# KatherLab/STAMP

Measured on AMD Instinct MI355X. Metric: tiles/sec encoded (224x224, ViT-L/14), higher is better.
Workload: dtype f16

## Files before the change

stamp_amd/csrc/attention_vit257.hip:

```cpp
#include "common.h"
#include <type_traits>

namespace amds {

constexpr int A7_KP = 256, A7_VS = 576;
constexpr int A7_K_BYTES = A7_KP * 128, A7_V_BYTES = 64 * A7_VS + 8 * 16, A7_T_BYTES = 3 * 64 * 4 + 128;
constexpr int A7_BUF = A7_K_BYTES + A7_V_BYTES + A7_T_BYTES;
constexpr int A7_PART = 68;
constexpr int A7_SCRATCH = 16 + 8 * 64 + 2 * 9 * A7_PART * 4;
constexpr int A7_OUT = 8 * 2048;
constexpr int A7_LDS = 2 * A7_BUF + A7_SCRATCH + A7_OUT;

#ifdef A7_TRACE
__device__ unsigned long long a7_trace[32 * 8 * 8];
#define A7_MARK(k)                                                                                            \
    do {                                                                                                      \
        if (blockIdx.x == 0 && lane == 0 && trace_it < 32) a7_trace[(trace_it * 8 + (k)) * 8 + wave] = __builtin_amdgcn_s_memtime(); \
    } while (0)
#else
#define A7_MARK(k) do { } while (0)
#endif

template <typename T>
__global__ void __launch_bounds__(512) attn_vit257_kernel(const T* __restrict__ qkv, T* __restrict__ out, int H, int n_items) {
    typedef typename Act<T>::vec8 vec8;
    typedef typename Act<T>::vec4 vec4;
    constexpr int Tn = 257, KP = A7_KP, VS = A7_VS;
    extern __shared__ __attribute__((aligned(16))) char smem[];
    char* sZero = smem + 2 * A7_BUF;
    char* sPw = sZero + 16;
    float* sPart = reinterpret_cast<float*>(sPw + 8 * 64);

    const int tid = threadIdx.x, lane = tid & 63;
    const int wave = __builtin_amdgcn_readfirstlane(tid >> 6);
    const int l31 = lane & 31, hi = lane >> 5;
    const int Dm = H * 64;
    const long ld = 3L * Dm;
    const float sc = 0.125f * 1.44269504088896340736f;
    const int swz = (l31 >> 1) & 7;

    struct Part { u32x4 k; u32x2 v0, v1; };
    Part pa, pb;
    T tq = (T)0.f, tk = (T)0.f, tv = (T)0.f;
    vec8 qn[4];
    const int ldb = (int)ld * 2;
    const int vu = tid >> 1, vhalf = tid & 1;
    const int voff_k = (tid >> 3) * ldb + Dm * 2 + (tid & 7) * 16;
    const int voff_v = (vu >> 3) * 2 * ldb + Dm * 4 + (vu & 7) * 16 + vhalf * 8;
    const int voff_q = (wave * 32 + l31) * ldb + hi * 16;
    const int lk_off = (tid >> 3) * 128 + (((tid & 7) ^ ((tid >> 4) & 7)) << 4);
    const int vk0 = (vu >> 3) * 2;
    const int lv_off = A7_K_BYTES + ((vu & 7) * 8 + vhalf * 4) * VS + (vu & 7) * 16 + ((vk0 & ~12) | ((vk0 & 4) << 1) | ((vk0 & 8) >> 1)) * 2;
    auto part_load = [&](Part& pt, __amdgpu_buffer_rsrc_t rs, int c) {
#if defined(A7_ABL) && (A7_ABL & 2)
        if (c >= 0) return;
#endif
        pt.k = __builtin_amdgcn_raw_buffer_load_b128(rs, voff_k, c * 64 * ldb, 0);
        pt.v0 = __builtin_amdgcn_raw_buffer_load_b64(rs, voff_v, c * 64 * ldb, 0);
        pt.v1 = __builtin_amdgcn_raw_buffer_load_b64(rs, voff_v, c * 64 * ldb + ldb, 0);
    };
    auto part_store = [&](const Part& pt, char* buf, int c) {
        *reinterpret_cast<u32x4*>(buf + lk_off + c * 64 * 128) = pt.k;
        typedef T vec4t __attribute__((ext_vector_type(4)));
        typedef T vec2 __attribute__((ext_vector_type(2)));
        const vec4t a = __builtin_bit_cast(vec4t, pt.v0), b2 = __builtin_bit_cast(vec4t, pt.v1);
#pragma unroll
        for (int e = 0; e < 4; ++e) {
            vec2 w;
            w[0] = a[e]; w[1] = b2[e];
            *reinterpret_cast<vec2*>(buf + lv_off + e * VS + c * 128) = w;
        }
    };
    auto rest_load = [&](__amdgpu_buffer_rsrc_t rs) {
#pragma unroll
        for (int ks = 0; ks < 4; ++ks) qn[ks] = __builtin_bit_cast(vec8, __builtin_amdgcn_raw_buffer_load_b128(rs, voff_q + ks * 32, 0, 0));
        tq = __builtin_bit_cast(T, __builtin_amdgcn_raw_buffer_load_b16(rs, lane * 2, KP * ldb, 0));
        tk = __builtin_bit_cast(T, __builtin_amdgcn_raw_buffer_load_b16(rs, lane * 2, KP * ldb + Dm * 2, 0));
        tv = __builtin_bit_cast(T, __builtin_amdgcn_raw_buffer_load_b16(rs, lane * 2, KP * ldb + Dm * 4, 0));
    };
    auto rest_store = [&](char* buf) {
        float* sT = reinterpret_cast<float*>(buf + A7_K_BYTES + A7_V_BYTES);
        if (tid < 64) {
            sT[tid] = Act<T>::to_f32(tk); sT[64 + tid] = Act<T>::to_f32(tv); sT[128 + tid] = Act<T>::to_f32(tq);
            reinterpret_cast<T*>(sT + 192)[tid] = tq;
        }
    };
    auto item_rsrc = [&](int item) {
        const int b = item / H, h = item - b * H;
        return __builtin_amdgcn_make_buffer_rsrc(const_cast<T*>(qkv + (long)b * Tn * ld + h * 64), 0, Tn * ldb, 0x00020000);
    };

    int item = blockIdx.x;
    if (item >= n_items) return;
    if (tid < 4) reinterpret_cast<float*>(sZero)[tid] = 0.f;
    auto merge_odd = [&](int pbuf, int it) {
        const float* pp = sPart + pbuf * 9 * A7_PART;
        float m = pp[64];
#pragma unroll
        for (int j = 1; j < 9; ++j) m = fmaxf(m, pp[j * A7_PART + 64]);
        float lsum = 0.f, ov = 0.f;
#pragma unroll
        for (int j = 0; j < 9; ++j) {
            const float w = __builtin_amdgcn_exp2f(pp[j * A7_PART + 64] - m);
            lsum = fmaf(w, pp[j * A7_PART + 65], lsum);
            ov = fmaf(w, pp[j * A7_PART + lane], ov);
        }
        const int b = it / H, h = it - b * H;
        out[((long)b * Tn + KP) * Dm + h * 64 + lane] = Act<T>::from_f32(ov / lsum);
    };
    {
        const __amdgpu_buffer_rsrc_t rs = item_rsrc(item);
        rest_load(rs);
#pragma unroll
        for (int c = 0; c < 4; c += 2) {
            part_load(pa, rs, c);
            part_load(pb, rs, c + 1);
            part_store(pa, smem, c);
            part_store(pb, smem, c + 1);
        }
        rest_store(smem);
    }
    vec8 qf[4];
#pragma unroll
    for (int ks = 0; ks < 4; ++ks) qf[ks] = qn[ks];
    __syncthreads();

    int cur = 0;
#ifdef A7_TRACE
    int trace_it = 0;
#endif
#pragma unroll 1
    for (; item < n_items; item += gridDim.x) {
        const int b = item / H, h = item - b * H;
        const char* sK = smem + cur * A7_BUF;
        const char* sVt = sK + A7_K_BYTES;
        const float* sKt = reinterpret_cast<const float*>(sK + A7_K_BYTES + A7_V_BYTES);
        const float* sVl = sKt + 64;
        const float* sQt = sKt + 128;
        const bool has_next = item + (int)gridDim.x < n_items;
        A7_MARK(0);
        if (wave == 0 && item != (int)blockIdx.x) merge_odd(cur ^ 1, item - (int)gridDim.x);
        const __amdgpu_buffer_rsrc_t nrs = item_rsrc(has_next ? item + (int)gridDim.x : item);
        A7_MARK(1);

        {
            f32x16 o[2];
#pragma unroll
            for (int dt = 0; dt < 2; ++dt)
#pragma unroll
                for (int r = 0; r < 16; ++r) o[dt][r] = 0.f;
            float mrun = -INFINITY, l = 0.f;
            const f32x16 zero16 = {0.f, 0.f, 0.f, 0.f, 0.f, 0.f, 0.f, 0.f, 0.f, 0.f, 0.f, 0.f, 0.f, 0.f, 0.f, 0.f};
            auto stage = [&](auto has_pv_c, auto has_qk_c, int c, float alpha_prev, f32x16 (&sc_)[2], vec8 (&pout)[2][2], const vec8 (&pprev)[2][2],
                             f32x16 (&sn)[2]) {
                constexpr bool HP = decltype(has_pv_c)::value, HQ = decltype(has_qk_c)::value;
                vec8 opnd[4];
                auto ld = [&](int i) {
                    if (i < 0 || i >= 16) return;
#if defined(A7_ABL) && (A7_ABL & 4)
                    if (i >= 0) { asm volatile("" : "+v"(opnd[i & 3])); return; }
#endif
                    if (i < 8) {
                        if (!HQ) return;
                        const int t = i & 1, ks = i >> 1;
                        opnd[i & 3] = *reinterpret_cast<const vec8*>(sK + (((c + 1) * 2 + t) * 32 + l31) * 128 + (((ks * 2 + hi) ^ swz) << 4));
                    } else {
                        if (!HP) return;
                        const int q = i - 8, t = q >> 2, ks = (q >> 1) & 1, dt = q & 1;
                        const int pos = ((c - 1) * 2 + t) * 32 + ks * 16 + hi * 8, d = dt * 32 + l31;
                        opnd[i & 3] = *reinterpret_cast<const vec8*>(sVt + d * VS + (d >> 3) * 16 + pos * 2);
                    }
                };
                auto mf = [&](int i) {
#if defined(A7_ABL) && (A7_ABL & 8)
                    if (i >= 0) { asm volatile("" : "+v"(sn[i & 1]), "+v"(o[i & 1]) : "v"(opnd[i & 3])); return; }
#endif
                    if (i < 8) {
                        if (!HQ) return;
                        const int t = i & 1, ks = i >> 1;
                        sn[t] = Act<T>::mfma32(opnd[i & 3], qf[ks], ks == 0 ? zero16 : sn[t]);
                    } else {
                        if (!HP) return;
                        const int q = i - 8, t = q >> 2, ks = (q >> 1) & 1, dt = q & 1;
                        o[dt] = Act<T>::mfma32(opnd[i & 3], pprev[t][ks], o[dt]);
                    }
                };
                float mx = -INFINITY, mnew = 0.f, alpha = 0.f, ls = 0.f;
#ifndef A7_LD_DIST
#define A7_LD_DIST 2
#endif
#pragma unroll
                for (int i = 0; i < A7_LD_DIST; ++i) ld(i);
#pragma unroll
                for (int sl = 0; sl < 16; ++sl) {
                    ld(sl + A7_LD_DIST);
                    mf(sl);
                    if (sl < 2) {
#pragma unroll
                        for (int f = 16 * sl; f < 16 * sl + 16; ++f) mx = fmaxf(mx, sc_[f >> 4][f & 15]);
                    }
                    if (sl == 2) {
                        mx = fmaxf(mx, __shfl_xor(mx, 32, 64));
                        mnew = fmaxf(mrun, mx * sc);
                        alpha = __builtin_amdgcn_exp2f(mrun - mnew);
                        mrun = mnew;
                    }
                    if ((sl == 2 || sl == 3) && HP) {
#pragma unroll
                        for (int r = 0; r < 16; ++r) o[sl - 2][r] *= alpha_prev;
                    }
                    if (sl >= 3 && sl < 14) {
#pragma unroll
                        for (int f = 3 * (sl - 3); f < 3 * (sl - 3) + 3 && f < 32; ++f) {
#if defined(A7_ABL) && (A7_ABL & 1)
                            const float pw = fmaf(sc_[f >> 4][f & 15], sc, -mnew);
#else
                            const float pw = __builtin_amdgcn_exp2f(fmaf(sc_[f >> 4][f & 15], sc, -mnew));
#endif
                            ls += pw;
                            pout[f >> 4][(f >> 3) & 1][f & 7] = Act<T>::from_f32(pw);
                        }
                    }
                    if (sl == 14) l = l * alpha + ls;
                    __builtin_amdgcn_sched_barrier(0);
                }
                return alpha;
            };
            typedef std::true_type Y;
            typedef std::false_type N_;
            char* nbuf = smem + (cur ^ 1) * A7_BUF;
            f32x16 sa[2], sb[2];
            vec8 p0[2][2], p1[2][2];
            part_load(pa, nrs, 0);
#pragma unroll
            for (int t = 0; t < 2; ++t) {
                sa[t] = zero16;
#pragma unroll
                for (int ks = 0; ks < 4; ++ks) {
                    const vec8 kf = *reinterpret_cast<const vec8*>(sK + (t * 32 + l31) * 128 + (((ks * 2 + hi) ^ swz) << 4));
                    sa[t] = Act<T>::mfma32(kf, qf[ks], sa[t]);
                }
            }
            __builtin_amdgcn_sched_barrier(0);
            part_load(pb, nrs, 1);
            __builtin_amdgcn_sched_barrier(0);
            const float al0 = stage(N_{}, Y{}, 0, 0.f, sa, p0, p1, sb);
            part_store(pa, nbuf, 0);
            part_load(pa, nrs, 2);
            __builtin_amdgcn_sched_barrier(0);
            const float al1 = stage(Y{}, Y{}, 1, al0, sb, p1, p0, sa);
            part_store(pb, nbuf, 1);
            part_load(pb, nrs, 3);
            __builtin_amdgcn_sched_barrier(0);
            const float al2 = stage(Y{}, Y{}, 2, al1, sa, p0, p1, sb);
            rest_load(nrs);
            __builtin_amdgcn_sched_barrier(0);
            const float al3 = stage(Y{}, N_{}, 3, al2, sb, p1, p0, sa);
#pragma unroll
            for (int dt = 0; dt < 2; ++dt)
#pragma unroll
                for (int r = 0; r < 16; ++r) o[dt][r] *= al3;
#pragma unroll
            for (int i = 0; i < 8; ++i) {
                const int t = i >> 2, ks = (i >> 1) & 1, dt = i & 1;
                const int pos = (6 + t) * 32 + ks * 16 + hi * 8, d = dt * 32 + l31;
                const vec8 vf = *reinterpret_cast<const vec8*>(sVt + d * VS + (d >> 3) * 16 + pos * 2);
                o[dt] = Act<T>::mfma32(vf, p1[t][ks], o[dt]);
            }
            A7_MARK(2);
            {
                float dot = 0.f;
#pragma unroll
                for (int ks = 0; ks < 4; ++ks) {
                    const f32x4 k0 = *reinterpret_cast<const f32x4*>(sKt + (ks * 2 + hi) * 8), k1 = *reinterpret_cast<const f32x4*>(sKt + (ks * 2 + hi) * 8 + 4);
#pragma unroll
                    for (int e = 0; e < 4; ++e) dot = fmaf(Act<T>::to_f32(qf[ks][e]), k0[e], fmaf(Act<T>::to_f32(qf[ks][4 + e]), k1[e], dot));
                }
                dot += __shfl_xor(dot, 32, 64);
                const float st = dot * sc, mnew = fmaxf(mrun, st);
                const float alpha = __builtin_amdgcn_exp2f(mrun - mnew), pt = __builtin_amdgcn_exp2f(st - mnew);
                mrun = mnew;
                l = l * alpha + (hi == 0 ? pt : 0.f);
#pragma unroll
                for (int dt = 0; dt < 2; ++dt)
#pragma unroll
                    for (int g = 0; g < 4; ++g) {
                        const f32x4 vv = *reinterpret_cast<const f32x4*>(sVl + dt * 32 + 8 * g + 4 * hi);
#pragma unroll
                        for (int e = 0; e < 4; ++e) o[dt][4 * g + e] = fmaf(o[dt][4 * g + e], alpha, pt * vv[e]);
                    }
            }
            l += __shfl_xor(l, 32, 64);
            const float inv = 1.0f / l;
            char* so = smem + 2 * A7_BUF + A7_SCRATCH + wave * 2048;
            T* obase = out + ((long)b * Tn + wave * 32) * Dm + h * 64;
#pragma unroll
            for (int r = 0; r < 2; ++r) {
                if ((l31 >> 4) == r) {
#pragma unroll
                    for (int dt = 0; dt < 2; ++dt)
#pragma unroll
                        for (int g = 0; g < 4; ++g) {
                            vec4 w;
#pragma unroll
                            for (int e = 0; e < 4; ++e) w[e] = Act<T>::from_f32(o[dt][4 * g + e] * inv);
                            *reinterpret_cast<vec4*>(so + (l31 & 15) * 128 + (((dt * 4 + g) ^ (l31 & 7)) << 4) + hi * 8) = w;
                        }
                }
                asm volatile("" ::: "memory");
#pragma unroll
                for (int k = 0; k < 2; ++k) {
                    const int row = k * 8 + (lane >> 3), c = lane & 7;
                    const u32x4 v = *reinterpret_cast<const u32x4*>(so + row * 128 + ((c ^ (row & 7)) << 4));
#if defined(A7_ABL) && (A7_ABL & 16)
                    if (n_items < 0)
#endif
                    *reinterpret_cast<u32x4*>(obase + (long)(r * 16 + row) * Dm + c * 8) = v;
                }
                asm volatile("" ::: "memory");
            }
        }

        A7_MARK(3);
        {
            const char* sQh = reinterpret_cast<const char*>(sKt + 192);
            const char* qsrc = l31 == 0 ? sQh + hi * 16 : sZero;
            const int qstep = l31 == 0 ? 32 : 0;
            f32x16 s1;
#pragma unroll
            for (int r = 0; r < 16; ++r) s1[r] = 0.f;
#pragma unroll
            for (int ks = 0; ks < 4; ++ks) {
                const vec8 qa = *reinterpret_cast<const vec8*>(qsrc + ks * qstep);
                const vec8 kf = *reinterpret_cast<const vec8*>(sK + (wave * 32 + l31) * 128 + (((ks * 2 + hi) ^ swz) << 4));
                s1 = Act<T>::mfma32(qa, kf, s1);
            }
            vec8 vfo[2][2];
#pragma unroll
            for (int ks = 0; ks < 2; ++ks)
#pragma unroll
                for (int dt = 0; dt < 2; ++dt) {
                    const int pos = wave * 32 + ks * 16 + hi * 8, d = dt * 32 + l31;
                    vfo[ks][dt] = *reinterpret_cast<const vec8*>(sVt + d * VS + (d >> 3) * 16 + pos * 2);
                }
            const float sv = hi == 0 ? s1[0] * sc : -INFINITY;
            const float mw = half_wave_max(sv);
            const float pk = hi == 0 ? __builtin_amdgcn_exp2f(sv - mw) : 0.f;
            const float lw = half_wave_sum(pk);
            char* pw = sPw + wave * 64;
            if (hi == 0) reinterpret_cast<T*>(pw)[(l31 & ~12) | ((l31 & 4) << 1) | ((l31 & 8) >> 1)] = Act<T>::from_f32(pk);
            asm volatile("" ::: "memory");
            const char* psrc = l31 == 0 ? pw + hi * 16 : sZero;
            f32x16 oq[2];
#pragma unroll
            for (int dt = 0; dt < 2; ++dt)
#pragma unroll
                for (int r = 0; r < 16; ++r) oq[dt][r] = 0.f;
#pragma unroll
            for (int ks = 0; ks < 2; ++ks) {
                const vec8 pf = *reinterpret_cast<const vec8*>(psrc + ks * qstep);
#pragma unroll
                for (int dt = 0; dt < 2; ++dt) oq[dt] = Act<T>::mfma32(vfo[ks][dt], pf, oq[dt]);
            }
            float* pp = sPart + (cur * 9 + wave) * A7_PART;
            if (l31 == 0) {
#pragma unroll
                for (int dt = 0; dt < 2; ++dt)
#pragma unroll
                    for (int g = 0; g < 4; ++g)
                        *reinterpret_cast<f32x4*>(pp + dt * 32 + 8 * g + 4 * hi) = f32x4{oq[dt][4 * g], oq[dt][4 * g + 1], oq[dt][4 * g + 2], oq[dt][4 * g + 3]};
                if (hi == 0) { pp[64] = mw; pp[65] = lw; }
            }
            if (wave == 1) {
                float* p8 = sPart + (cur * 9 + 8) * A7_PART;
                float st = half_wave_sum(sQt[lane] * sKt[lane]);
                st = (st + __shfl_xor(st, 32, 64)) * sc;
                p8[lane] = sVl[lane];
                if (lane == 0) { p8[64] = st; p8[65] = 1.0f; }
            }
        }

        A7_MARK(4);
        {
            char* nbuf = smem + (cur ^ 1) * A7_BUF;
            part_store(pa, nbuf, 2);
            part_store(pb, nbuf, 3);
            rest_store(nbuf);
#pragma unroll
            for (int ks = 0; ks < 4; ++ks) qf[ks] = qn[ks];
        }
        A7_MARK(5);
        __syncthreads();
        A7_MARK(6);
        cur ^= 1;
#ifdef A7_TRACE
        ++trace_it;
#endif
    }
    if (wave == 0) merge_odd(cur ^ 1, item - (int)gridDim.x);
}


template <typename T>
static int launch_attn257(const void* qkv, void* out, int B, int H, hipStream_t st) {
    auto kern = attn_vit257_kernel<T>;
    static bool attr_set = false;
    if (!attr_set) {
        AMDS_HIP(hipFuncSetAttribute(reinterpret_cast<const void*>(kern), hipFuncAttributeMaxDynamicSharedMemorySize, A7_LDS));
        attr_set = true;
    }
    const int n_cus = device_cu_count();
    AMDS_REQUIRE(n_cus > 0, "attention: cannot read the device's multiprocessor count");
    const int n_items = B * H;
    hipLaunchKernelGGL(kern, dim3(min(n_items, n_cus)), dim3(512), A7_LDS, st, (const T*)qkv, (T*)out, H, n_items);
    AMDS_LAUNCH_CHECK("attn_vit257_kernel");
    return AMDS_OK;
}

int attention_vit257(const void* qkv, void* out, int B, int H, int dtype, hipStream_t st) {
    return dtype == AMDS_F16 ? launch_attn257<f16>(qkv, out, B, H, st) : launch_attn257<bf16>(qkv, out, B, H, st);
}

}
```

Measured before the change: 6057.

## Load K/V straight to LDS and read V transposed with ds_read_b64_tr_b16

Replaces the register-staged K/V prefetch, which loaded into VGPRs and then wrote a manually transposed V layout to LDS, with direct buffer-to-LDS loads (bufl16) using an XOR-swizzled row layout for both K and V. The PV MFMA operands are then fetched with ds_read_b64_tr_b16 transpose reads, using per-lane addresses that flip between the double buffers each iteration. This removes the VGPR staging and the scalar-pair transpose stores, and with them some register pressure and LDS write traffic. In exchange it adds explicit vmcnt/lgkmcnt waits before each barrier and inline-asm reads that each wait on lgkmcnt(0), which may serialize LDS latency inside the pipelined stages.

```diff
diff --git a/stamp_amd/csrc/attention_vit257.hip b/stamp_amd/csrc/attention_vit257.hip
--- a/stamp_amd/csrc/attention_vit257.hip
+++ b/stamp_amd/csrc/attention_vit257.hip
@@ -3,8 +3,8 @@
 
 namespace amds {
 
-constexpr int A7_KP = 256, A7_VS = 576;
-constexpr int A7_K_BYTES = A7_KP * 128, A7_V_BYTES = 64 * A7_VS + 8 * 16, A7_T_BYTES = 3 * 64 * 4 + 128;
+constexpr int A7_KP = 256;
+constexpr int A7_K_BYTES = A7_KP * 128, A7_V_BYTES = A7_KP * 128, A7_T_BYTES = 3 * 64 * 4 + 128;
 constexpr int A7_BUF = A7_K_BYTES + A7_V_BYTES + A7_T_BYTES;
 constexpr int A7_PART = 68;
 constexpr int A7_SCRATCH = 16 + 8 * 64 + 2 * 9 * A7_PART * 4;
@@ -21,11 +21,22 @@
 #define A7_MARK(k) do { } while (0)
 #endif
 
+__device__ __forceinline__ int a7_swz(int row) { return (((row >> 1) & 1) << 2) | ((row >> 2) & 3); }
+
+#define A7_TR8(out, a00, a01, a10, a11, imm)                                                                                              \
+    asm volatile("ds_read_b64_tr_b16 %0, %8 offset:%12\n\tds_read_b64_tr_b16 %1, %10 offset:%12\n\t"                                  \
+                 "ds_read_b64_tr_b16 %2, %9 offset:%12\n\tds_read_b64_tr_b16 %3, %11 offset:%12\n\t"                                   \
+                 "ds_read_b64_tr_b16 %4, %8 offset:%13\n\tds_read_b64_tr_b16 %5, %10 offset:%13\n\t"                                   \
+                 "ds_read_b64_tr_b16 %6, %9 offset:%13\n\tds_read_b64_tr_b16 %7, %11 offset:%13\n\ts_waitcnt lgkmcnt(0)"               \
+                 : "=&v"(out[0]), "=&v"(out[1]), "=&v"(out[2]), "=&v"(out[3]), "=&v"(out[4]), "=&v"(out[5]), "=&v"(out[6]), "=&v"(out[7])  \
+                 : "v"(a00), "v"(a01), "v"(a10), "v"(a11), "n"(imm), "n"((imm) + 2048)                                                  \
+                 : "memory")
+
 template <typename T>
 __global__ void __launch_bounds__(512) attn_vit257_kernel(const T* __restrict__ qkv, T* __restrict__ out, int H, int n_items) {
     typedef typename Act<T>::vec8 vec8;
     typedef typename Act<T>::vec4 vec4;
-    constexpr int Tn = 257, KP = A7_KP, VS = A7_VS;
+    constexpr int Tn = 257, KP = A7_KP;
     extern __shared__ __attribute__((aligned(16))) char smem[];
     char* sZero = smem + 2 * A7_BUF;
     char* sPw = sZero + 16;
@@ -37,39 +48,20 @@
     const int Dm = H * 64;
     const long ld = 3L * Dm;
     const float sc = 0.125f * 1.44269504088896340736f;
-    const int swz = (l31 >> 1) & 7;
-
-    struct Part { u32x4 k; u32x2 v0, v1; };
-    Part pa, pb;
+    const int swz = a7_swz(l31);
+
     T tq = (T)0.f, tk = (T)0.f, tv = (T)0.f;
     vec8 qn[4];
     const int ldb = (int)ld * 2;
-    const int vu = tid >> 1, vhalf = tid & 1;
-    const int voff_k = (tid >> 3) * ldb + Dm * 2 + (tid & 7) * 16;
-    const int voff_v = (vu >> 3) * 2 * ldb + Dm * 4 + (vu & 7) * 16 + vhalf * 8;
+    const int drow = wave * 8 + (lane >> 3);
+    const int voff_kv = drow * ldb + (((lane & 7) ^ a7_swz(drow)) << 4);
     const int voff_q = (wave * 32 + l31) * ldb + hi * 16;
-    const int lk_off = (tid >> 3) * 128 + (((tid & 7) ^ ((tid >> 4) & 7)) << 4);
-    const int vk0 = (vu >> 3) * 2;
-    const int lv_off = A7_K_BYTES + ((vu & 7) * 8 + vhalf * 4) * VS + (vu & 7) * 16 + ((vk0 & ~12) | ((vk0 & 4) << 1) | ((vk0 & 8) >> 1)) * 2;
-    auto part_load = [&](Part& pt, __amdgpu_buffer_rsrc_t rs, int c) {
+    auto part_dma = [&](__amdgpu_buffer_rsrc_t rs, char* buf, int c) {
 #if defined(A7_ABL) && (A7_ABL & 2)
         if (c >= 0) return;
 #endif
-        pt.k = __builtin_amdgcn_raw_buffer_load_b128(rs, voff_k, c * 64 * ldb, 0);
-        pt.v0 = __builtin_amdgcn_raw_buffer_load_b64(rs, voff_v, c * 64 * ldb, 0);
-        pt.v1 = __builtin_amdgcn_raw_buffer_load_b64(rs, voff_v, c * 64 * ldb + ldb, 0);
-    };
-    auto part_store = [&](const Part& pt, char* buf, int c) {
-        *reinterpret_cast<u32x4*>(buf + lk_off + c * 64 * 128) = pt.k;
-        typedef T vec4t __attribute__((ext_vector_type(4)));
-        typedef T vec2 __attribute__((ext_vector_type(2)));
-        const vec4t a = __builtin_bit_cast(vec4t, pt.v0), b2 = __builtin_bit_cast(vec4t, pt.v1);
-#pragma unroll
-        for (int e = 0; e < 4; ++e) {
-            vec2 w;
-            w[0] = a[e]; w[1] = b2[e];
-            *reinterpret_cast<vec2*>(buf + lv_off + e * VS + c * 128) = w;
-        }
+        bufl16(rs, buf + (c * 8 + wave) * 1024, voff_kv, c * 64 * ldb + Dm * 2);
+        bufl16(rs, buf + A7_K_BYTES + (c * 8 + wave) * 1024, voff_kv, c * 64 * ldb + Dm * 4);
     };
     auto rest_load = [&](__amdgpu_buffer_rsrc_t rs) {
 #pragma unroll
@@ -112,18 +104,30 @@
         const __amdgpu_buffer_rsrc_t rs = item_rsrc(item);
         rest_load(rs);
 #pragma unroll
-        for (int c = 0; c < 4; c += 2) {
-            part_load(pa, rs, c);
-            part_load(pb, rs, c + 1);
-            part_store(pa, smem, c);
-            part_store(pb, smem, c + 1);
-        }
+        for (int c = 0; c < 4; ++c) part_dma(rs, smem, c);
         rest_store(smem);
     }
     vec8 qf[4];
 #pragma unroll
     for (int ks = 0; ks < 4; ++ks) qf[ks] = qn[ks];
+    asm volatile("s_waitcnt vmcnt(0) lgkmcnt(0)" ::: "memory");
     __syncthreads();
+    unsigned tra[2][2];
+    {
+        const int i16 = lane & 15, gd = (lane >> 4) & 1;
+#pragma unroll
+        for (int w = 0; w < 2; ++w)
+#pragma unroll
+            for (int dt = 0; dt < 2; ++dt) {
+                const int row = hi * 4 + w * 8 + (i16 >> 2);
+                const int lc = dt * 4 + gd * 2 + ((i16 & 3) >> 1);
+                tra[w][dt] = (unsigned)(size_t)smem + A7_K_BYTES + row * 128 + ((lc ^ a7_swz(row)) << 4) + (i16 & 1) * 8;
+            }
+    }
+    int flip = A7_BUF;
+#if defined(A7_ABL) && (A7_ABL & 32)
+    if (wave >= 4) __builtin_amdgcn_s_setprio(1);
+#endif
 
     int cur = 0;
 #ifdef A7_TRACE
@@ -133,7 +137,6 @@
     for (; item < n_items; item += gridDim.x) {
         const int b = item / H, h = item - b * H;
         const char* sK = smem + cur * A7_BUF;
-        const char* sVt = sK + A7_K_BYTES;
         const float* sKt = reinterpret_cast<const float*>(sK + A7_K_BYTES + A7_V_BYTES);
         const float* sVl = sKt + 64;
         const float* sQt = sKt + 128;
@@ -150,30 +153,30 @@
 #pragma unroll
                 for (int r = 0; r < 16; ++r) o[dt][r] = 0.f;
             float mrun = -INFINITY, l = 0.f;
+            auto vt_frag = [&](const u32x2 (&f)[8], int ks, int dt) {
+                return __builtin_bit_cast(vec8, u32x4{f[ks * 4 + dt * 2][0], f[ks * 4 + dt * 2][1], f[ks * 4 + dt * 2 + 1][0], f[ks * 4 + dt * 2 + 1][1]});
+            };
             const f32x16 zero16 = {0.f, 0.f, 0.f, 0.f, 0.f, 0.f, 0.f, 0.f, 0.f, 0.f, 0.f, 0.f, 0.f, 0.f, 0.f, 0.f};
-            auto stage = [&](auto has_pv_c, auto has_qk_c, int c, float alpha_prev, f32x16 (&sc_)[2], vec8 (&pout)[2][2], const vec8 (&pprev)[2][2],
+            auto stage = [&](auto has_pv_c, auto has_qk_c, auto c_, float alpha_prev, f32x16 (&sc_)[2], vec8 (&pout)[2][2], const vec8 (&pprev)[2][2],
                              f32x16 (&sn)[2]) {
                 constexpr bool HP = decltype(has_pv_c)::value, HQ = decltype(has_qk_c)::value;
+                constexpr int c = decltype(c_)::value;
                 vec8 opnd[4];
+                u32x2 tv[2][8];
                 auto ld = [&](int i) {
-                    if (i < 0 || i >= 16) return;
+                    if (i < 0 || i >= 8) return;
 #if defined(A7_ABL) && (A7_ABL & 4)
                     if (i >= 0) { asm volatile("" : "+v"(opnd[i & 3])); return; }
 #endif
-                    if (i < 8) {
-                        if (!HQ) return;
-                        const int t = i & 1, ks = i >> 1;
-                        opnd[i & 3] = *reinterpret_cast<const vec8*>(sK + (((c + 1) * 2 + t) * 32 + l31) * 128 + (((ks * 2 + hi) ^ swz) << 4));
-                    } else {
-                        if (!HP) return;
-                        const int q = i - 8, t = q >> 2, ks = (q >> 1) & 1, dt = q & 1;
-                        const int pos = ((c - 1) * 2 + t) * 32 + ks * 16 + hi * 8, d = dt * 32 + l31;
-                        opnd[i & 3] = *reinterpret_cast<const vec8*>(sVt + d * VS + (d >> 3) * 16 + pos * 2);
-                    }
+                    if (!HQ) return;
+                    const int t = i & 1, ks = i >> 1;
+                    opnd[i & 3] = *reinterpret_cast<const vec8*>(sK + (((c + 1) * 2 + t) * 32 + l31) * 128 + (((ks * 2 + hi) ^ swz) << 4));
                 };
+                const unsigned a00 = tra[0][0], a01 = tra[0][1], a10 = tra[1][0], a11 = tra[1][1];
+                constexpr int vimm = HP ? (c - 1) * 2 * 4096 : 0;
                 auto mf = [&](int i) {
 #if defined(A7_ABL) && (A7_ABL & 8)
-                    if (i >= 0) { asm volatile("" : "+v"(sn[i & 1]), "+v"(o[i & 1]) : "v"(opnd[i & 3])); return; }
+                    if (i >= 0) { asm volatile("" : "+v"(sn[i & 1]), "+v"(o[i & 1]) : "v"(opnd[i & 3]), "v"(tv[(i >> 2) & 1][i & 7])); return; }
 #endif
                     if (i < 8) {
                         if (!HQ) return;
@@ -182,18 +185,30 @@
                     } else {
                         if (!HP) return;
                         const int q = i - 8, t = q >> 2, ks = (q >> 1) & 1, dt = q & 1;
-                        o[dt] = Act<T>::mfma32(opnd[i & 3], pprev[t][ks], o[dt]);
+                        o[dt] = Act<T>::mfma32(vt_frag(tv[t], ks, dt), pprev[t][ks], o[dt]);
                     }
                 };
                 float mx = -INFINITY, mnew = 0.f, alpha = 0.f, ls = 0.f;
 #ifndef A7_LD_DIST
 #define A7_LD_DIST 2
 #endif
+#ifndef A7_LV0
+#define A7_LV0 6
+#define A7_LV1 10
+#endif
 #pragma unroll
                 for (int i = 0; i < A7_LD_DIST; ++i) ld(i);
 #pragma unroll
                 for (int sl = 0; sl < 16; ++sl) {
                     ld(sl + A7_LD_DIST);
+                    if constexpr (HP) {
+#if defined(A7_ABL) && (A7_ABL & 4)
+                        if (sl == A7_LV0 || sl == A7_LV1) asm volatile("" : "+v"(tv[sl == A7_LV1][0]), "+v"(tv[sl == A7_LV1][2]), "+v"(tv[sl == A7_LV1][4]), "+v"(tv[sl == A7_LV1][6]) : "v"(a00), "v"(a01), "v"(a10), "v"(a11));
+#else
+                        if (sl == A7_LV0) A7_TR8(tv[0], a00, a01, a10, a11, vimm);
+                        if (sl == A7_LV1) A7_TR8(tv[1], a00, a01, a10, a11, vimm + 4096);
+#endif
+                    }
                     mf(sl);
                     if (sl < 2) {
 #pragma unroll
@@ -231,7 +246,7 @@
             char* nbuf = smem + (cur ^ 1) * A7_BUF;
             f32x16 sa[2], sb[2];
             vec8 p0[2][2], p1[2][2];
-            part_load(pa, nrs, 0);
+            part_dma(nrs, nbuf, 0);
 #pragma unroll
             for (int t = 0; t < 2; ++t) {
                 sa[t] = zero16;
@@ -242,30 +257,32 @@
                 }
             }
             __builtin_amdgcn_sched_barrier(0);
-            part_load(pb, nrs, 1);
+            part_dma(nrs, nbuf, 1);
             __builtin_amdgcn_sched_barrier(0);
-            const float al0 = stage(N_{}, Y{}, 0, 0.f, sa, p0, p1, sb);
-            part_store(pa, nbuf, 0);
-            part_load(pa, nrs, 2);
+            const float al0 = stage(N_{}, Y{}, std::integral_constant<int, 0>{}, 0.f, sa, p0, p1, sb);
+            part_dma(nrs, nbuf, 2);
             __builtin_amdgcn_sched_barrier(0);
-            const float al1 = stage(Y{}, Y{}, 1, al0, sb, p1, p0, sa);
-            part_store(pb, nbuf, 1);
-            part_load(pb, nrs, 3);
+            const float al1 = stage(Y{}, Y{}, std::integral_constant<int, 1>{}, al0, sb, p1, p0, sa);
+            part_dma(nrs, nbuf, 3);
             __builtin_amdgcn_sched_barrier(0);
-            const float al2 = stage(Y{}, Y{}, 2, al1, sa, p0, p1, sb);
+            const float al2 = stage(Y{}, Y{}, std::integral_constant<int, 2>{}, al1, sa, p0, p1, sb);
             rest_load(nrs);
             __builtin_amdgcn_sched_barrier(0);
-            const float al3 = stage(Y{}, N_{}, 3, al2, sb, p1, p0, sa);
+            const float al3 = stage(Y{}, N_{}, std::integral_constant<int, 3>{}, al2, sb, p1, p0, sa);
 #pragma unroll
             for (int dt = 0; dt < 2; ++dt)
 #pragma unroll
                 for (int r = 0; r < 16; ++r) o[dt][r] *= al3;
-#pragma unroll
-            for (int i = 0; i < 8; ++i) {
-                const int t = i >> 2, ks = (i >> 1) & 1, dt = i & 1;
-                const int pos = (6 + t) * 32 + ks * 16 + hi * 8, d = dt * 32 + l31;
-                const vec8 vf = *reinterpret_cast<const vec8*>(sVt + d * VS + (d >> 3) * 16 + pos * 2);
-                o[dt] = Act<T>::mfma32(vf, p1[t][ks], o[dt]);
+            {
+                u32x2 tl[2][8];
+                const unsigned a00 = tra[0][0], a01 = tra[0][1], a10 = tra[1][0], a11 = tra[1][1];
+                A7_TR8(tl[0], a00, a01, a10, a11, 6 * 4096);
+                A7_TR8(tl[1], a00, a01, a10, a11, 7 * 4096);
+#pragma unroll
+                for (int i = 0; i < 8; ++i) {
+                    const int t = i >> 2, ks = (i >> 1) & 1, dt = i & 1;
+                    o[dt] = Act<T>::mfma32(vt_frag(tl[t], ks, dt), p1[t][ks], o[dt]);
+                }
             }
             A7_MARK(2);
             {
@@ -335,14 +352,12 @@
                 const vec8 kf = *reinterpret_cast<const vec8*>(sK + (wave * 32 + l31) * 128 + (((ks * 2 + hi) ^ swz) << 4));
                 s1 = Act<T>::mfma32(qa, kf, s1);
             }
-            vec8 vfo[2][2];
-#pragma unroll
-            for (int ks = 0; ks < 2; ++ks)
-#pragma unroll
-                for (int dt = 0; dt < 2; ++dt) {
-                    const int pos = wave * 32 + ks * 16 + hi * 8, d = dt * 32 + l31;
-                    vfo[ks][dt] = *reinterpret_cast<const vec8*>(sVt + d * VS + (d >> 3) * 16 + pos * 2);
-                }
+            u32x2 tvo[8];
+            {
+                const unsigned wo = wave * 4096;
+                const unsigned a00 = tra[0][0] + wo, a01 = tra[0][1] + wo, a10 = tra[1][0] + wo, a11 = tra[1][1] + wo;
+                A7_TR8(tvo, a00, a01, a10, a11, 0);
+            }
             const float sv = hi == 0 ? s1[0] * sc : -INFINITY;
             const float mw = half_wave_max(sv);
             const float pk = hi == 0 ? __builtin_amdgcn_exp2f(sv - mw) : 0.f;
@@ -360,7 +375,8 @@
             for (int ks = 0; ks < 2; ++ks) {
                 const vec8 pf = *reinterpret_cast<const vec8*>(psrc + ks * qstep);
 #pragma unroll
-                for (int dt = 0; dt < 2; ++dt) oq[dt] = Act<T>::mfma32(vfo[ks][dt], pf, oq[dt]);
+                for (int dt = 0; dt < 2; ++dt)
+                    oq[dt] = Act<T>::mfma32(__builtin_bit_cast(vec8, u32x4{tvo[ks * 4 + dt * 2][0], tvo[ks * 4 + dt * 2][1], tvo[ks * 4 + dt * 2 + 1][0], tvo[ks * 4 + dt * 2 + 1][1]}), pf, oq[dt]);
             }
             float* pp = sPart + (cur * 9 + wave) * A7_PART;
             if (l31 == 0) {
@@ -383,13 +399,14 @@
         A7_MARK(4);
         {
             char* nbuf = smem + (cur ^ 1) * A7_BUF;
-            part_store(pa, nbuf, 2);
-            part_store(pb, nbuf, 3);
             rest_store(nbuf);
 #pragma unroll
             for (int ks = 0; ks < 4; ++ks) qf[ks] = qn[ks];
         }
+        tra[0][0] += flip; tra[0][1] += flip; tra[1][0] += flip; tra[1][1] += flip;
+        flip = -flip;
         A7_MARK(5);
+        asm volatile("s_waitcnt vmcnt(0) lgkmcnt(0)" ::: "memory");
         __syncthreads();
         A7_MARK(6);
         cur ^= 1;
```

After: 6050. Within noise of the previous version (-0.1%).
